# hrnr/map-merge

Measured on AMD Instinct MI355X. Metric: map-pairs/sec (normals+FPFH+SAC-IA+ICP, end to end incl. per-map features), higher is better.
Workload: dtype f32; 1 GPU; 16 maps x 500000 raw pts, FPFH + SAC_IA + ICP refine, 120 pairs; parallelism=one mm3d_estimate_maps_transforms call, 16 streams inside the library, points_after_filter_mean=406681, keypoints_mean=15692

## Files before the change

include/mm3d.h:

```cpp
#ifndef MM3D_H_
#define MM3D_H_

#include <stddef.h>
#include <stdint.h>

#ifdef __cplusplus
extern "C" {
#endif

typedef enum {
  MM3D_OK = 0,
  MM3D_EINVAL = -1,
  MM3D_EDEVICE = -2,
  MM3D_ENOMEM = -3,
  MM3D_EUNSUPPORTED = -4,
  MM3D_ECAPACITY = -5
} mm3d_status;

typedef enum { MM3D_DESC_PFH = 0, MM3D_DESC_PFHRGB, MM3D_DESC_FPFH, MM3D_DESC_RSD, MM3D_DESC_SHOT, MM3D_DESC_SC3D } mm3d_descriptor;
typedef enum { MM3D_KP_SIFT = 0, MM3D_KP_HARRIS } mm3d_keypoint;
typedef enum { MM3D_EST_MATCHING = 0, MM3D_EST_SAC_IA } mm3d_estimation_method;
typedef enum { MM3D_ICP_POINT_TO_POINT = 0, MM3D_ICP_POINT_TO_PLANE = 1 } mm3d_icp_method;

const char *mm3d_descriptor_name(int d);
// ... 71 lines not shown
int mm3d_debug_feature_lds_cap(int cap);
void mm3d_debug_feature_overflow(long long out[8], int reset);
void mm3d_debug_sacia_stats(long long out[4], int reset, int collect);
int mm3d_debug_desc_knn(mm3d_ctx *ctx, const float *a, size_t na, const float *b, size_t nb, int dim, int k, int *idx, float *d2);
typedef struct mm3d_nn_search_info {
  float max_d2;
  float rmax;
  float cell;
  float origin[3];
  int dims[3];
  int max_ring;
  int n_items;
} mm3d_nn_search_info;
int mm3d_debug_nn_search(mm3d_ctx *ctx, const mm3d_cloud *source, const mm3d_cloud *target, const float T[16], double range,
                         int convention, int split, int *idx, float *d2, mm3d_nn_search_info *info);
void mm3d_srand(mm3d_ctx *ctx, unsigned seed);
int mm3d_set_streams(mm3d_ctx *ctx, int n_streams);
int mm3d_get_streams(const mm3d_ctx *ctx);
int mm3d_last_run_stage_seconds(const mm3d_ctx *ctx, double *features_s, double *total_s);
int mm3d_last_run_device_seconds(const mm3d_ctx *ctx, double *exchange_s, double *pairs_s, double *gather_s);
size_t mm3d_last_run_map_sizes(const mm3d_ctx *ctx, size_t *points, size_t *keypoints, size_t capacity);
int mm3d_set_map_cache(mm3d_ctx *ctx, int max_maps);
int mm3d_get_map_cache(const mm3d_ctx *ctx);
void mm3d_map_cache_clear(mm3d_ctx *ctx);
int mm3d_map_cache_stats(const mm3d_ctx *ctx, long long out[6], int reset);
int mm3d_set_icp_method(mm3d_ctx *ctx, int method);
int mm3d_get_icp_method(const mm3d_ctx *ctx);
typedef enum { MM3D_ALIGN_SAC_IA = 0, MM3D_ALIGN_PREREJECTIVE = 1 } mm3d_align_method;
typedef struct mm3d_alignment_options {
  int method;
// ... 422 lines not shown
```

map-merge_amd/__init__.py:

```python
from __future__ import annotations

import ctypes as C
import enum
import os
import subprocess

import numpy as np

_HERE = os.path.dirname(os.path.abspath(__file__))
LIB_PATH = os.environ.get("MM3D_LIB") or os.path.join(_HERE, "libmm3d.so")

POINT = np.dtype([("x", "<f4"), ("y", "<f4"), ("z", "<f4"), ("rgba", "<u4")])
NORMAL = np.dtype([("nx", "<f4"), ("ny", "<f4"), ("nz", "<f4"), ("curvature", "<f4")])
CORR = np.dtype([("index_query", "<i4"), ("index_match", "<i4"), ("distance", "<f4")])
PAIR = np.dtype([("source_idx", "<u8"), ("target_idx", "<u8"), ("transform", "<f4", (16,)),
                 ("confidence", "<f8"), ("icp_iterations", "<i4"), ("n_correspondences", "<i4"),
                 ("n_inliers", "<i4"), ("icp_correspondences", "<i4")])


class Mm3dError(RuntimeError):
    def __init__(self, status, msg):
        super().__init__(f"mm3d status {status}: {msg}")
        self.status = status

# ... 1236 lines not shown
        self._ck(lib().mm3d_debug_wave_primitives(self._h, int(op), v.ctypes.data_as(C.c_void_p), len(v),
                                                  new.ctypes.data_as(C.c_void_p), old.ctypes.data_as(C.c_void_p)))
        return new, old

    def debugNnSearch(self, source_points, target_points, transform, range, convention, split):
        n = len(source_points)
        idx = np.zeros(max(n, 1), dtype=np.int32)
        d2 = np.zeros(max(n, 1), dtype=np.float32)
        t = _T(transform)
        info = NnSearchInfo()
        self._ck(lib().mm3d_debug_nn_search(self._h, source_points._h, target_points._h, t.ctypes.data_as(C.c_void_p),
                                            C.c_double(range), int(convention), int(split), idx.ctypes.data_as(C.c_void_p),
                                            d2.ctypes.data_as(C.c_void_p), C.byref(info)))
        return idx[:n], d2[:n], info.as_dict()

    def debugColorGradients(self, points, normals, options=None, **kw):
        o = options if options is not None else IcpColorOptions(**kw)
        n = len(points)
        out = np.zeros((max(n, 1), 4), dtype=np.float32)
        self._ck(lib().mm3d_debug_color_gradients(self._h, points._h, normals._h, C.byref(o), out.ctypes.data_as(C.c_void_p)))
        return out[:n]

    def debugIcpRejection(self, source_points, target_points, transform, max_correspondence_distance, options=None, split=1, **kw):
        o = options if options is not None else IcpRejectionOptions(**kw)
        n = len(source_points)
        idx = np.zeros(max(n, 1), dtype=np.int32)
        d2 = np.zeros(max(n, 1), dtype=np.float32)
        kept = np.zeros(max(n, 1), dtype=np.uint8)
        t = _T(transform)
        st = IcpRejectionStats()
# ... 247 lines not shown
```

map-merge_amd/csrc/device_util.hpp:

```cpp
#pragma once

#include <hip/hip_runtime.h>

#include <type_traits>

#include "libm_exact.hpp"
#include "types.hpp"

namespace mm3d {

constexpr int kWave = 64;
constexpr int kXcds = 8;

__device__ __forceinline__ unsigned xcd_remap(unsigned bid, unsigned nblocks)
{
  unsigned q = nblocks / kXcds, r = nblocks % kXcds;
  unsigned xcd = bid % kXcds, k = bid / kXcds;
  unsigned base = xcd < r ? xcd * (q + 1) : r * (q + 1) + (xcd - r) * q;
  return base + k;
}

__device__ __forceinline__ unsigned f2ord(float f)
{
  unsigned u = __float_as_uint(f);
// ... 14 lines not shown
__device__ __forceinline__ float dist2(float ax, float ay, float az, float bx, float by, float bz)
{
  float dx = ax - bx, dy = ay - by, dz = az - bz;
  return __fadd_rn(__fadd_rn(__fmul_rn(dx, dx), __fmul_rn(dy, dy)), __fmul_rn(dz, dz));
}

__device__ __forceinline__ float3 xform(const float *T, float x, float y, float z)
{
  float3 r;
  r.x = __fadd_rn(__fadd_rn(__fadd_rn(__fmul_rn(T[0], x), __fmul_rn(T[4], y)), __fmul_rn(T[8], z)), T[12]);
  r.y = __fadd_rn(__fadd_rn(__fadd_rn(__fmul_rn(T[1], x), __fmul_rn(T[5], y)), __fmul_rn(T[9], z)), T[13]);
  r.z = __fadd_rn(__fadd_rn(__fadd_rn(__fmul_rn(T[2], x), __fmul_rn(T[6], y)), __fmul_rn(T[10], z)), T[14]);
  return r;
}

__device__ __forceinline__ int cell_floor(float v, float mn, float inv)
{
  float f = floorf((v - mn) * inv);
  f = fminf(fmaxf(f, -1048576.0f), 1048576.0f);
  return (int)f;
}

__device__ __forceinline__ int clampi(int v, int lo, int hi) { return v < lo ? lo : (v > hi ? hi : v); }

template <class F>
__device__ __forceinline__ void for_each_candidate(const GridView &g, float qx, float qy, float qz, float r, F &&f)
{
  const float ri = r * 1.0001f + 1e-4f;
  int x0 = clampi(cell_floor(qx - ri, g.minx, g.inv), 0, g.dx - 1);
  int x1 = clampi(cell_floor(qx + ri, g.minx, g.inv), 0, g.dx - 1);
  int y0 = cell_floor(qy - ri, g.miny, g.inv), y1 = cell_floor(qy + ri, g.miny, g.inv);
  int z0 = cell_floor(qz - ri, g.minz, g.inv), z1 = cell_floor(qz + ri, g.minz, g.inv);
  if (cell_floor(qx + ri, g.minx, g.inv) < 0 || cell_floor(qx - ri, g.minx, g.inv) > g.dx - 1) return;
  y0 = y0 < 0 ? 0 : y0; z0 = z0 < 0 ? 0 : z0;
  y1 = y1 > g.dy - 1 ? g.dy - 1 : y1; z1 = z1 > g.dz - 1 ? g.dz - 1 : z1;
  for (int z = z0; z <= z1; ++z)
    for (int y = y0; y <= y1; ++y) {
      const int row = (z * g.dy + y) * g.dx;
// ... 368 lines not shown
```

map-merge_amd/csrc/filters.hip:

```cpp
#include <algorithm>
#include <climits>

#include "lattice.hpp"
#include "scan_fused.hpp"

namespace mm3d {

__global__ void k_voxel_keys(const float4 *__restrict__ pts, int n, float inv, int minbx, int minby, int minbz,
                             int mul1, int mul2, uint32_t *__restrict__ keys, uint32_t *__restrict__ vals)
{
  int i = blockIdx.x * blockDim.x + threadIdx.x;
  if (i >= n) return;
  float4 p = pts[i];
  vals[i] = (uint32_t)i;
  if (!(isfinite(p.x) && isfinite(p.y) && isfinite(p.z))) { keys[i] = 0xFFFFFFFFu; return; }
  int ijk0 = (int)(lattice_index(p.x, inv) - (float)minbx);
  int ijk1 = (int)(lattice_index(p.y, inv) - (float)minby);
  int ijk2 = (int)(lattice_index(p.z, inv) - (float)minbz);
  keys[i] = (uint32_t)(ijk0 + ijk1 * mul1 + ijk2 * mul2);
}

struct VoxelHeadLoad {
  const uint32_t *keys; int n;
  __device__ __forceinline__ int operator()(size_t j) const
  {
    if (j >= (size_t)n) return 0;
    const uint32_t k = keys[j];
    return (k != 0xFFFFFFFFu && (j == 0 || keys[j - 1] != k)) ? 1 : 0;
  }
};
struct VoxelStartStore {
  int n; int *starts; int *n_voxels;
  __device__ __forceinline__ void operator()(size_t j, int prefix, int v) const
  {
// ... 102 lines not shown
{
  auto *in = const_cast<mm3d_cloud *>(in_);
  cloud_bbox(c, in);
  const int n = (int)in->n;
  if (n == 0 || in->n_finite == 0) return cloud_from_device(c, DevBuf<float4>(c, 0), 0);
  const float leaf = (float)resolution;
  const VoxelSetup vs = voxel_setup(in, leaf);
  const float inv = vs.inv;
  if (vs.overflow) {
    DevBuf<float4> copy(c, in->n);
    MM3D_HIP(hipMemcpyAsync(copy.get(), in->pts.get(), in->n * 16, hipMemcpyDeviceToDevice, c->stream));
    return cloud_from_device(c, std::move(copy), in->n);
  }
  const int *min_b = vs.min_b, *div_b = vs.div_b;
  const int mul1 = div_b[0], mul2 = div_b[0] * div_b[1];
  DevBuf<uint32_t> keys(c, n), vals(c, n), keys2(c, n), vals2(c, n);
  MM3D_LAUNCH(c, "voxel_keys", n * 24.0, k_voxel_keys, dim3(div_up(n, 256)), dim3(256), 0, in->pts.get(), n, inv,
              min_b[0], min_b[1], min_b[2], mul1, mul2, keys.get(), vals.get());
  DevBuf<int> too_long(c, 1);
  counting_sort_pairs_u32(c, keys.get(), n, (uint64_t)div_b[0] * (uint64_t)div_b[1] * (uint64_t)div_b[2], keys2.get(), vals2.get(),
                          too_long.get(), in->n_finite == in->n);
  const size_t bound = in->n_finite;
  DevBuf<int> starts(c, (size_t)n + 1);
  static const unsigned cblocks_cap = [] { const char *e = getenv("MM3D_VOXEL_BLOCKS"); return e ? (unsigned)std::max(1, atoi(e)) : 240u; }();
  const unsigned cblocks = std::min<unsigned>(div_up(bound, 256), cblocks_cap);
  DevBuf<unsigned> ctl(c, 16 + 8 * (size_t)cblocks);
  DevBuf<float4> out(c, bound);
  const size_t ctl_bytes = (16 + 8 * (size_t)cblocks) * sizeof(unsigned);
  unsigned *h = (unsigned *)c->pin(64 + ctl_bytes);
  for (int attempt = 0; attempt < 2; ++attempt) {
    scan_fused(c, "voxel_starts", n * 12.0, (size_t)n + 1, VoxelHeadLoad{keys2.get(), n}, VoxelStartStore{n, starts.get(), (int *)ctl.get()});
    MM3D_LAUNCH(c, "voxel_centroid", in->n_finite * 32.0, k_voxel_centroid, dim3(cblocks), dim3(256), 0, in->pts.get(),
                (const uint32_t *)vals2.get(), (const int *)starts.get(), (int *)ctl.get(), attempt == 0 ? (const int *)too_long.get() : (const int *)nullptr, (int)in->n_finite, 2.0f * leaf,
                out.get(), ctl.get() + 16);
    MM3D_HIP(hipMemcpyAsync(h + 16, ctl.get(), ctl_bytes, hipMemcpyDeviceToHost, c->stream));
    MM3D_HIP(hipMemcpyAsync(h + 15, too_long.get(), sizeof(int), hipMemcpyDeviceToHost, c->stream));
    c->sync();
    if (attempt == 1 || !h[15]) break;
    sort_pairs_u32(c, keys.get(), keys2.get(), vals.get(), vals2.get(), n, 32);
  }
  const size_t nvox = h[16];
  refit_points(c, out, nvox, bound);
  mm3d_cloud *res = cloud_from_device(c, std::move(out), nvox);
  unsigned box[8];
  box_of_slots(h + 32, cblocks, box);
  cloud_set_bbox(res, box);
  if (h[17] == 0) res->voxel_leaf = leaf;
  c->settle();
  return res;
}

__global__ void __launch_bounds__(256)
k_radius_count(GridView g, float radius, float thr, int need, int *__restrict__ keep )
{
// ... 76 lines not shown
```

map-merge_amd/csrc/grid.hip:

```cpp
#include <hip/hip_runtime.h>

#include <cstring>

#include <rocprim/rocprim.hpp>

#include "device_util.hpp"
#include "scan_fused.hpp"

namespace mm3d {


__global__ void __launch_bounds__(256)
k_scan_int(const int *__restrict__ in, int *__restrict__ out, size_t n, unsigned long long *status, unsigned *ticket,
           unsigned ticket_base, unsigned epoch)
{
  __shared__ unsigned s_tile;
  __shared__ int s_wave[4];
  __shared__ int s_prefix;
  if (threadIdx.x == 0) s_tile = atomicAdd(ticket, 1u) - ticket_base;
  __syncthreads();
  const size_t tile = s_tile;
  const size_t base = tile * kScanTile + (size_t)threadIdx.x * kScanItems;
  int v[kScanItems];
  int sum = 0;
// ... 504 lines not shown
  MM3D_HIP(hipMemcpyAsync(h, g.nb_start.get() + nc, sizeof(int), hipMemcpyDeviceToHost, c->stream));
  c->sync();
  const size_t total = (size_t)h[0];
  g.nb_pts = DevBuf<float4>(c, total ? total : 1);
  if (total) {
    MM3D_LAUNCH(c, "grid_nblists", total * 32.0, k_nb_fill, dim3(div_up(nc, 4)), dim3(256), 0, (const int *)g.cell_start.get(),
                (const float4 *)g.sorted.get(), g.dims[0], g.dims[1], g.dims[2], R, (const int *)g.nb_start.get(), g.nb_pts.get());
    MM3D_LAUNCH(c, "grid_nblists", total * 32.0, k_nb_sort, dim3(div_up(nc, 4)), dim3(256), 0, g.mn[0], g.mn[1], g.mn[2], g.cell,
                g.dims[0], g.dims[1], g.dims[2], (const int *)g.nb_start.get(), g.nb_pts.get());
  }
  g.nb_R = R;
  c->settle();
}

__global__ void k_hilbert_keys(const float4 *__restrict__ pts, int n, float minx, float miny, float minz, float inv,
                               uint32_t *__restrict__ keys, uint32_t *__restrict__ vals, int *__restrict__ counts, uint32_t *__restrict__ ranks)
{
  const int i = blockIdx.x * blockDim.x + threadIdx.x;
  if (i >= n) return;
  const float4 p = pts[i];
  vals[i] = (uint32_t)i;
  if (!(isfinite(p.x) && isfinite(p.y) && isfinite(p.z))) { keys[i] = 0xFFFFFFFFu; return; }
  unsigned x = (unsigned)clampi(cell_floor(p.x, minx, inv), 0, 1023);
  unsigned y = (unsigned)clampi(cell_floor(p.y, miny, inv), 0, 1023);
  const unsigned z = (unsigned)clampi(cell_floor(p.z, minz, inv), 0, 1023);
  unsigned d = 0;
  for (unsigned sft = 512; sft > 0; sft >>= 1) {
    const unsigned rx = (x & sft) ? 1u : 0u, ry = (y & sft) ? 1u : 0u;
    d += sft * sft * ((3u * rx) ^ ry);
    if (ry == 0) {
      if (rx == 1) { x = 1023u - x; y = 1023u - y; }
      const unsigned t = x; x = y; y = t;
    }
  }
  const uint32_t key = (d << 10) | z;
  keys[i] = key;
  if (counts) ranks[i] = (uint32_t)atomicAdd(&counts[key >> 10], 1);
}

// ... 2 lines not shown
  const int j = blockIdx.x * blockDim.x + threadIdx.x;
  if (j >= n) return;
  const uint32_t i = order[j];
  float4 p = pts[i];
  p.w = __int_as_float((int)i);
  out[j] = p;
}

struct ItemHeadLoad {
  const uint32_t *keys; int n; const int *inert;
  __device__ __forceinline__ bool head(size_t j) const { return j < (size_t)n && (j == 0 || (keys[j] >> 16) != (keys[j - 1] >> 16) || (j & 63) == 0); }
  __device__ __forceinline__ int operator()(size_t j) const { return (inert && *inert) ? 0 : (head(j) ? 1 : 0); }
};
struct ItemFillStore {
  const uint32_t *keys; int n; int2 *items; int *n_items; const int *inert;
  __device__ __forceinline__ void operator()(size_t j, int prefix, int v) const
  {
    if (j == (size_t)n) { *n_items = prefix; return; }
    if (!v) return;
    const ItemHeadLoad h{keys, n, nullptr};
    int cnt = 1;
    while (cnt < 64 && j + cnt < (size_t)n && !h.head(j + cnt)) ++cnt;
    items[prefix] = make_int2((int)j, cnt);
  }
  __device__ __forceinline__ void done() const {}
};

constexpr int kCountSortBinMax = 1024;
__global__ void k_cs_count(const uint32_t *__restrict__ keys, int n, uint32_t divisor, int *__restrict__ counts, uint32_t *__restrict__ ranks)
{
  const int i = blockIdx.x * blockDim.x + threadIdx.x;
  if (i >= n) return;
  const uint32_t key = keys[i];
  if (key == 0xFFFFFFFFu) return;
  ranks[i] = (uint32_t)atomicAdd(&counts[key / divisor], 1);
}
__global__ void k_cs_scatter(const uint32_t *__restrict__ keys, const uint32_t *__restrict__ ranks, const int *__restrict__ bin_start, int n,
                             uint32_t divisor, int *__restrict__ slots, int *__restrict__ too_long)
{
  const int i = blockIdx.x * blockDim.x + threadIdx.x;
  if (i >= n) return;
  const uint32_t key = keys[i];
  if (key == 0xFFFFFFFFu) return;
  const uint32_t bin = key / divisor;
  const int b = bin_start[bin];
  slots[b + (int)ranks[i]] = i;
  if (bin_start[bin + 1] - b > kCountSortBinMax) *too_long = 1;
}
__global__ void k_cs_place(const uint32_t *__restrict__ keys, const int *__restrict__ bin_start, const int *__restrict__ slots, int n,
                           uint32_t divisor, const int *__restrict__ too_long, uint32_t *__restrict__ keys_out, uint32_t *__restrict__ idx_out)
{
  const int i = blockIdx.x * blockDim.x + threadIdx.x;
  if (i >= n || *too_long) return;
  const uint32_t key = keys[i];
  if (key == 0xFFFFFFFFu) return;
  const uint32_t bin = key / divisor;
  const int b = bin_start[bin], e = bin_start[bin + 1];
  int r = 0;
  for (int j = b; j < e; ++j) {
    const int o = slots[j];
    const uint32_t ko = keys[o];
    r += (ko < key || (ko == key && o < i)) ? 1 : 0;
  }
  keys_out[b + r] = key;
  idx_out[b + r] = (uint32_t)i;
}

void counting_sort_pairs_u32(Context *c, const uint32_t *keys, int n, uint64_t key_range, uint32_t *keys_out, uint32_t *idx_out,
                             int *too_long, bool no_invalid_keys)
{
  uint32_t divisor = (uint32_t)((key_range + ((uint64_t)1 << 22) - 1) >> 22);
  if (divisor == 0) divisor = 1;
  const int nbins = (int)(key_range / divisor) + 1;
  DevBuf<int> counts(c, (size_t)nbins + 1), bin_start(c, (size_t)nbins + 1), slots(c, (size_t)n);
  DevBuf<uint32_t> ranks(c, (size_t)n);
  MM3D_HIP(hipMemsetAsync(counts.get(), 0, ((size_t)nbins + 1) * sizeof(int), c->stream));
  MM3D_HIP(hipMemsetAsync(too_long, 0, sizeof(int), c->stream));
  if (!no_invalid_keys) MM3D_HIP(hipMemsetAsync(keys_out, 0xFF, (size_t)n * sizeof(uint32_t), c->stream));
  MM3D_LAUNCH(c, "count_sort", n * 12.0, k_cs_count, dim3(div_up(n, 256)), dim3(256), 0, keys, n, divisor, counts.get(), ranks.get());
  exclusive_scan_int(c, counts.get(), bin_start.get(), (size_t)nbins + 1);
  MM3D_LAUNCH(c, "count_sort", n * 16.0, k_cs_scatter, dim3(div_up(n, 256)), dim3(256), 0, keys, (const uint32_t *)ranks.get(),
              (const int *)bin_start.get(), n, divisor, slots.get(), too_long);
  MM3D_LAUNCH(c, "count_sort", n * 24.0, k_cs_place, dim3(div_up(n, 256)), dim3(256), 0, keys, (const int *)bin_start.get(),
              (const int *)slots.get(), n, divisor, (const int *)too_long, keys_out, idx_out);
}

constexpr int kHilColumns = 1 << 20;
constexpr int kHilColumnMax = 1024;
__global__ void k_hil_scatter(const uint32_t *__restrict__ keys, const uint32_t *__restrict__ ranks, const int *__restrict__ col_start, int n,
                              int *__restrict__ slots, int *__restrict__ too_long)
{
  const int i = blockIdx.x * blockDim.x + threadIdx.x;
  if (i >= n) return;
  const uint32_t key = keys[i];
  if (key == 0xFFFFFFFFu) return;
  const int b = col_start[key >> 10];
  slots[b + (int)ranks[i]] = i;
  if (col_start[(key >> 10) + 1] - b > kHilColumnMax) *too_long = 1;
}
__global__ void k_hil_place(const float4 *__restrict__ pts, const uint32_t *__restrict__ keys, const int *__restrict__ col_start,
                            const int *__restrict__ slots, int n, const int *__restrict__ too_long, float4 *__restrict__ out,
                            uint32_t *__restrict__ out_keys)
{
  const int i = blockIdx.x * blockDim.x + threadIdx.x;
  if (i >= n || *too_long) return;
  const uint32_t key = keys[i];
  if (key == 0xFFFFFFFFu) return;
  const int b = col_start[key >> 10], e = col_start[(key >> 10) + 1];
  int r = 0;
  for (int j = b; j < e; ++j) {
    const int o = slots[j];
    const uint32_t ko = keys[o];
    r += (ko < key || (ko == key && o < i)) ? 1 : 0;
  }
  float4 p = pts[i];
  p.w = __int_as_float(i);
  out[b + r] = p;
  out_keys[b + r] = key;
}

void cloud_hilbert(Context *c, const mm3d_cloud *cl_, float min_cell)
{
  auto *cl = const_cast<mm3d_cloud *>(cl_);
  std::lock_guard<std::recursive_mutex> lk(cl->cache_mu);
  cloud_bbox(c, cl);
  const int n = (int)cl->n_finite;
  if (cl->hil_pts.get() || n == 0) return;
  const int total = (int)cl->n;
  float ext = 0.f;
  for (int a = 0; a < 3; ++a) ext = std::fmax(ext, cl->bmax[a] - cl->bmin[a]);
  const float cell = std::fmax(std::fmax(0.25f, min_cell), ext / 1023.0f);
  DevBuf<uint32_t> keys(c, total), vals(c, total), keys2(c, total);
  cl->hil_pts = DevBuf<float4>(c, n);
  DevBuf<int> counts(c, kHilColumns + 2), col_start(c, kHilColumns + 1), slots(c, n);
  DevBuf<uint32_t> ranks(c, total);
  MM3D_HIP(hipMemsetAsync(counts.get(), 0, (kHilColumns + 2) * sizeof(int), c->stream));
  const DevPtr<int> too_long{counts.get() + kHilColumns + 1};
  MM3D_LAUNCH(c, "hilbert_keys", total * 36.0, k_hilbert_keys, dim3(div_up(total, 256)), dim3(256), 0, cl->pts.get(), total,
              cl->bmin[0], cl->bmin[1], cl->bmin[2], 1.0f / cell, keys.get(), vals.get(), counts.get(), ranks.get());
  exclusive_scan_int(c, counts.get(), col_start.get(), kHilColumns + 1);
  MM3D_LAUNCH(c, "hilbert_sort", total * 16.0, k_hil_scatter, dim3(div_up(total, 256)), dim3(256), 0, (const uint32_t *)keys.get(),
              (const uint32_t *)ranks.get(), (const int *)col_start.get(), total, slots.get(), too_long.get());
  MM3D_LAUNCH(c, "hilbert_sort", total * 44.0, k_hil_place, dim3(div_up(total, 256)), dim3(256), 0, cl->pts.get(),
              (const uint32_t *)keys.get(), (const int *)col_start.get(), (const int *)slots.get(), total, (const int *)too_long.get(),
              cl->hil_pts.get(), keys2.get());
  const size_t max_items = (size_t)n / 64 + 16384 + 2;
  cl->wave_items = DevBuf<int2>(c, max_items);
  DevBuf<int> n_items_dev(c, 1);
  int *h = (int *)c->pin(64);
  for (int attempt = 0; attempt < 2; ++attempt) {
    const int *inert = attempt == 0 ? (const int *)too_long.get() : nullptr;
    scan_fused(c, "hilbert_items", n * 20.0, (size_t)n + 1, ItemHeadLoad{keys2.get(), n, inert},
               ItemFillStore{keys2.get(), n, cl->wave_items.get(), n_items_dev.get(), inert});
    MM3D_HIP(hipMemcpyAsync(h, n_items_dev.get(), sizeof(int), hipMemcpyDeviceToHost, c->stream));
    MM3D_HIP(hipMemcpyAsync(h + 1, too_long.get(), sizeof(int), hipMemcpyDeviceToHost, c->stream));
    c->sync();
    if (attempt == 1 || !h[1]) break;
    DevBuf<uint32_t> vals2(c, total);
    sort_pairs_u32(c, keys.get(), keys2.get(), vals.get(), vals2.get(), total, 32);
// ... 73 lines not shown
}

int snb_cu_count(int device)
{
  static std::mutex mu;
  static std::map<int, int> cache;
  std::lock_guard<std::mutex> lk(mu);
  auto it = cache.find(device);
  if (it != cache.end()) return it->second;
  int n = 0;
  if (hipDeviceGetAttribute(&n, hipDeviceAttributeMultiprocessorCount, device) != hipSuccess || n <= 0) n = 256;
  cache[device] = n;
  return n;
}

}
```

map-merge_amd/csrc/scan_fused.hpp:

```cpp
#pragma once

#include "device_util.hpp"

namespace mm3d {

struct BoxAcc {
  float mn[3] = {INFINITY, INFINITY, INFINITY}, mx[3] = {-INFINITY, -INFINITY, -INFINITY};
  int cnt = 0;
  __device__ __forceinline__ void add(const float4 &p)
  {
    mn[0] = fminf(mn[0], p.x); mn[1] = fminf(mn[1], p.y); mn[2] = fminf(mn[2], p.z);
    mx[0] = fmaxf(mx[0], p.x); mx[1] = fmaxf(mx[1], p.y); mx[2] = fmaxf(mx[2], p.z);
    ++cnt;
  }
  template <bool kSlot>
  __device__ __forceinline__ void flush_impl(unsigned *box)
  {
    __shared__ float s_mn[4][3], s_mx[4][3];
    __shared__ int s_cnt[4];
#pragma unroll
    for (int a = 0; a < 3; ++a) { mn[a] = wave_min_f(mn[a]); mx[a] = wave_max_f(mx[a]); }
    const int total = wave_sum(cnt);
    const int lane = threadIdx.x & 63, wave = (threadIdx.x >> 6) & 3;
    if (lane == 0) {
// ... 23 lines not shown
  __device__ __forceinline__ void flush(unsigned *box) { flush_impl<false>(box); }
  __device__ __forceinline__ void flush_slot(unsigned *slots) { flush_impl<true>(slots + 8 * (size_t)blockIdx.x); }
};
inline void box_of_slots(const unsigned *slots, unsigned blocks, unsigned *box)
{
  for (int a = 0; a < 3; ++a) { box[a] = 0xFFFFFFFFu; box[3 + a] = 0u; }
  box[6] = 0u;
  for (unsigned b = 0; b < blocks; ++b) {
    const unsigned *s = slots + 8 * (size_t)b;
    for (int a = 0; a < 3; ++a) { box[a] = s[a] < box[a] ? s[a] : box[a]; box[3 + a] = s[3 + a] > box[3 + a] ? s[3 + a] : box[3 + a]; }
    box[6] += s[6];
  }
}
constexpr unsigned kBoxInit[8] = {0xFFFFFFFFu, 0xFFFFFFFFu, 0xFFFFFFFFu, 0u, 0u, 0u, 0u, 0u};

template <class Load, class Store>
__global__ void __launch_bounds__(256)
k_scan_fused(size_t n, unsigned long long *status, unsigned *ticket, unsigned ticket_base, unsigned epoch, Load load, Store store)
{
  __shared__ unsigned s_tile;
  __shared__ int s_wave[4];
  __shared__ int s_prefix;
  if (threadIdx.x == 0) s_tile = atomicAdd(ticket, 1u) - ticket_base;
  __syncthreads();
  const size_t tile = s_tile;
  const size_t base = tile * kScanTile + (size_t)threadIdx.x * kScanItems;
  int v[kScanItems];
  int sum = 0;
#pragma unroll
  for (int k = 0; k < kScanItems; ++k) v[k] = base + k < n ? load(base + k) : 0;
#pragma unroll
  for (int k = 0; k < kScanItems; ++k) sum += v[k];
  const int lane = threadIdx.x & 63, wave = threadIdx.x >> 6;
  const int incl = wave_scan_incl(sum);
  if (lane == kWave - 1) s_wave[wave] = incl;
  __syncthreads();
  int wave_off = 0;
  for (int w = 0; w < wave; ++w) wave_off += s_wave[w];
  const int total = s_wave[0] + s_wave[1] + s_wave[2] + s_wave[3];
  if (wave == 0) {
    const unsigned long long tag = (unsigned long long)epoch << 34;
    if (lane == 0 && tile > 0)
      __hip_atomic_store(&status[tile], tag | (1ull << 32) | (unsigned)total, __ATOMIC_RELAXED, __HIP_MEMORY_SCOPE_AGENT);
    int prefix = 0;
    for (long long hi = (long long)tile - 1; hi >= 0; hi -= kWave) {
      const long long t = hi - lane;
      unsigned long long w = 2ull << 32;
      if (t >= 0) {
// ... 1 lines not shown
        while ((w >> 34) != epoch || ((w >> 32) & 3u) == 0u);
      }
      const unsigned long long is_prefix = ballot(((w >> 32) & 3u) == 2u);
      const int first = __ffsll((long long)is_prefix) - 1;
      const int take = (first < 0 || lane <= first) ? (int)(unsigned)(w & 0xffffffffull) : 0;
      prefix += wave_sum(take);
      if (first >= 0) break;
    }
    if (lane == 0) {
      __hip_atomic_store(&status[tile], tag | (2ull << 32) | (unsigned)(prefix + total), __ATOMIC_RELAXED, __HIP_MEMORY_SCOPE_AGENT);
      s_prefix = prefix;
    }
  }
  __syncthreads();
  int run = s_prefix + wave_off + incl - sum;
#pragma unroll
  for (int k = 0; k < kScanItems; ++k) {
    if (base + k < n) store(base + k, run, v[k]);
    run += v[k];
  }
  store.done();
}

template <class Load, class Store>
void scan_fused(Context *c, const char *name, double bytes, size_t n, Load load, Store store)
{
  if (n == 0) return;
  const ScanLaunchState st = scan_prepare(c, n);
  MM3D_LAUNCH(c, name, bytes, (k_scan_fused<Load, Store>), dim3(st.tiles), dim3(256), 0, n, st.status, st.ticket, st.ticket_base, st.epoch, load, store);
}

}
```

map-merge_amd/csrc/types.hpp:

```cpp
#pragma once

#include "common.hpp"

namespace mm3d {
struct DeviceSet;
struct IcpMethodBase;
struct AlignMethodBase;
struct KeypointSourceBase;
struct CoarseMethodBase;
struct ConfidenceMethodBase;
struct EstimatorMethodBase;
struct IcpSamplerBase;
struct OutlierFilterBase;
struct ClusterFilterBase;
struct SmootherBase;
struct PlaneFilterBase;

struct StageSelection {
  const IcpMethodBase *icp = nullptr;
  const AlignMethodBase *align = nullptr;
  const KeypointSourceBase *keypoints = nullptr;
  const IcpMethodBase *refine = nullptr;
  const CoarseMethodBase *coarse = nullptr;
  const ConfidenceMethodBase *confidence = nullptr;
// ... 220 lines not shown
void cloud_hilbert(Context *c, const mm3d_cloud *cl, float min_cell = 0.25f);
mm3d_cloud *cloud_from_device(Context *c, DevBuf<float4> &&pts, size_t n);
mm3d_cloud *cloud_from_memory(Context *c, const void *src, size_t n, size_t stride, size_t rgba_off);
void cloud_download(Context *c, const mm3d_cloud *cl, void *dst, size_t stride, size_t rgba_off);
const std::vector<float4> &cloud_host(Context *c, const mm3d_cloud *cl, bool wait = true);
size_t compact_points(Context *c, const float4 *in, const int *flags, size_t n, DevBuf<float4> &out, unsigned *box_host = nullptr);
void cloud_set_bbox(mm3d_cloud *cl, const unsigned box[7]);
void refit_points(Context *c, DevBuf<float4> &out, size_t m, size_t bound);
mm3d_cloud *cloud_of_kept(Context *c, const mm3d_cloud *in, const int *flags, bool inherits_leaf, size_t *kept = nullptr);
void exclusive_scan_int(Context *c, const int *in, int *out, size_t n);
constexpr int kScanItems = 16, kScanTile = 256 * kScanItems;
struct ScanLaunchState { unsigned long long *status; unsigned *ticket; unsigned ticket_base, epoch, tiles; };
ScanLaunchState scan_prepare(Context *c, size_t n);
void counting_sort_pairs_u32(Context *c, const uint32_t *keys, int n, uint64_t key_range, uint32_t *keys_out, uint32_t *idx_out,
                             int *too_long, bool no_invalid_keys = false);
void sort_pairs_u32(Context *c, const uint32_t *kin, uint32_t *kout, const uint32_t *vin, uint32_t *vout,
                    size_t n, int end_bit);

mm3d_cloud *downsample(Context *c, const mm3d_cloud *in, double resolution);
bool downsample_is_identity(Context *c, const mm3d_cloud *in, double resolution);
mm3d_cloud *remove_outliers(Context *c, const mm3d_cloud *in, double radius, int min_neighbours);
mm3d_cloud *transform_concat(Context *c, const mm3d_cloud *const *clouds, size_t n, const float *T);

mm3d_normals *compute_normals(Context *c, const mm3d_cloud *in, double radius);

mm3d_cloud *detect_keypoints_sift(Context *c, const mm3d_cloud *points, double min_scale, int nr_octaves, int nr_scales, double min_contrast,
                                  double normals_radius = 0.0, mm3d_normals **normals_out = nullptr, float grid_cell_hint = 0.0f);
void normals_of_items(Context *c, const mm3d_cloud *in, const Grid &g, double radius, const int *ov_items, const int *ov_count_dev, int n_overflow,
                      float4 *out);

// ... 205 lines not shown
```

Baseline: 1464 map-pairs/s.

## Fuse voxel key counting, store key pairs in sort slots, precompute item spans

```diff
diff --git a/include/mm3d.h b/include/mm3d.h
--- a/include/mm3d.h
+++ b/include/mm3d.h
@@ -109,6 +109,9 @@
 } mm3d_nn_search_info;
 int mm3d_debug_nn_search(mm3d_ctx *ctx, const mm3d_cloud *source, const mm3d_cloud *target, const float T[16], double range,
                          int convention, int split, int *idx, float *d2, mm3d_nn_search_info *info);
+int mm3d_debug_hilbert_order(mm3d_ctx *ctx, const mm3d_cloud *cloud, float min_cell, int *order, int *items, size_t items_cap, int *n_items);
+int mm3d_debug_counting_sort(mm3d_ctx *ctx, const uint32_t *keys, size_t n, uint64_t key_range, int no_invalid_keys, uint32_t *keys_out,
+                             uint32_t *idx_out, int *too_long);
 void mm3d_srand(mm3d_ctx *ctx, unsigned seed);
 int mm3d_set_streams(mm3d_ctx *ctx, int n_streams);
 int mm3d_get_streams(const mm3d_ctx *ctx);
diff --git a/map-merge_amd/__init__.py b/map-merge_amd/__init__.py
--- a/map-merge_amd/__init__.py
+++ b/map-merge_amd/__init__.py
@@ -1274,6 +1274,26 @@
                                             d2.ctypes.data_as(C.c_void_p), C.byref(info)))
         return idx[:n], d2[:n], info.as_dict()
 
+    def debugHilbertOrder(self, points, min_cell=0.25):
+        n = len(points)
+        cap = n // 64 + 16386
+        order = np.full(max(n, 1), -1, dtype=np.int32)
+        items = np.zeros((cap, 2), dtype=np.int32)
+        m = C.c_int(0)
+        self._ck(lib().mm3d_debug_hilbert_order(self._h, points._h, C.c_float(min_cell), order.ctypes.data_as(C.c_void_p),
+                                                items.ctypes.data_as(C.c_void_p), C.c_size_t(cap), C.byref(m)))
+        order = order[:n]
+        return order[order >= 0], items[:m.value]
+
+    def debugCountingSort(self, keys, key_range, no_invalid_keys=False):
+        k = np.ascontiguousarray(keys, dtype=np.uint32)
+        ko, io = np.zeros(len(k), dtype=np.uint32), np.zeros(len(k), dtype=np.uint32)
+        tl = C.c_int(0)
+        self._ck(lib().mm3d_debug_counting_sort(self._h, k.ctypes.data_as(C.c_void_p), C.c_size_t(len(k)), C.c_uint64(int(key_range)),
+                                                int(bool(no_invalid_keys)), ko.ctypes.data_as(C.c_void_p), io.ctypes.data_as(C.c_void_p),
+                                                C.byref(tl)))
+        return ko, io, bool(tl.value)
+
     def debugColorGradients(self, points, normals, options=None, **kw):
         o = options if options is not None else IcpColorOptions(**kw)
         n = len(points)
diff --git a/map-merge_amd/csrc/device_util.hpp b/map-merge_amd/csrc/device_util.hpp
--- a/map-merge_amd/csrc/device_util.hpp
+++ b/map-merge_amd/csrc/device_util.hpp
@@ -52,14 +52,14 @@
   return r;
 }
 
-__device__ __forceinline__ int cell_floor(float v, float mn, float inv)
+__host__ __device__ __forceinline__ int cell_floor(float v, float mn, float inv)
 {
   float f = floorf((v - mn) * inv);
   f = fminf(fmaxf(f, -1048576.0f), 1048576.0f);
   return (int)f;
 }
 
-__device__ __forceinline__ int clampi(int v, int lo, int hi) { return v < lo ? lo : (v > hi ? hi : v); }
+__host__ __device__ __forceinline__ int clampi(int v, int lo, int hi) { return v < lo ? lo : (v > hi ? hi : v); }
 
 template <class F>
 __device__ __forceinline__ void for_each_candidate(const GridView &g, float qx, float qy, float qz, float r, F &&f)
diff --git a/map-merge_amd/csrc/filters.hip b/map-merge_amd/csrc/filters.hip
--- a/map-merge_amd/csrc/filters.hip
+++ b/map-merge_amd/csrc/filters.hip
@@ -18,6 +18,21 @@
   int ijk1 = (int)(lattice_index(p.y, inv) - (float)minby);
   int ijk2 = (int)(lattice_index(p.z, inv) - (float)minbz);
   keys[i] = (uint32_t)(ijk0 + ijk1 * mul1 + ijk2 * mul2);
+}
+
+__global__ void k_voxel_keys_count(const float4 *__restrict__ pts, int n, float inv, int minbx, int minby, int minbz, int mul1, int mul2,
+                                   uint32_t divisor, uint32_t *__restrict__ keys, int *__restrict__ counts, uint32_t *__restrict__ ranks)
+{
+  int i = blockIdx.x * blockDim.x + threadIdx.x;
+  if (i >= n) return;
+  float4 p = pts[i];
+  if (!(isfinite(p.x) && isfinite(p.y) && isfinite(p.z))) { keys[i] = 0xFFFFFFFFu; return; }
+  int ijk0 = (int)(lattice_index(p.x, inv) - (float)minbx);
+  int ijk1 = (int)(lattice_index(p.y, inv) - (float)minby);
+  int ijk2 = (int)(lattice_index(p.z, inv) - (float)minbz);
+  const uint32_t key = (uint32_t)(ijk0 + ijk1 * mul1 + ijk2 * mul2);
+  keys[i] = key;
+  if (key != 0xFFFFFFFFu) ranks[i] = (uint32_t)atomicAdd(&counts[key / divisor], 1);
 }
 
 struct VoxelHeadLoad {
@@ -150,12 +165,21 @@
   }
   const int *min_b = vs.min_b, *div_b = vs.div_b;
   const int mul1 = div_b[0], mul2 = div_b[0] * div_b[1];
+  const uint64_t key_range = (uint64_t)div_b[0] * (uint64_t)div_b[1] * (uint64_t)div_b[2];
+#if MM3D_VOXEL_FUSED
+  DevBuf<uint32_t> keys(c, n), keys2(c, n), vals2(c, n);
+  const CountingSort cs = counting_sort_begin(c, n, key_range);
+  const DevPtr<int> too_long{cs.too_long()};
+  MM3D_LAUNCH(c, "voxel_keys", n * 28.0, k_voxel_keys_count, dim3(div_up(n, 256)), dim3(256), 0, in->pts.get(), n, inv,
+              min_b[0], min_b[1], min_b[2], mul1, mul2, cs.divisor, keys.get(), cs.counts.get(), cs.ranks.get());
+  counting_sort_finish(c, cs, keys.get(), n, keys2.get(), vals2.get(), in->n_finite == in->n);
+#else
   DevBuf<uint32_t> keys(c, n), vals(c, n), keys2(c, n), vals2(c, n);
   MM3D_LAUNCH(c, "voxel_keys", n * 24.0, k_voxel_keys, dim3(div_up(n, 256)), dim3(256), 0, in->pts.get(), n, inv,
               min_b[0], min_b[1], min_b[2], mul1, mul2, keys.get(), vals.get());
   DevBuf<int> too_long(c, 1);
-  counting_sort_pairs_u32(c, keys.get(), n, (uint64_t)div_b[0] * (uint64_t)div_b[1] * (uint64_t)div_b[2], keys2.get(), vals2.get(),
-                          too_long.get(), in->n_finite == in->n);
+  counting_sort_pairs_u32(c, keys.get(), n, key_range, keys2.get(), vals2.get(), too_long.get(), in->n_finite == in->n);
+#endif
   const size_t bound = in->n_finite;
   DevBuf<int> starts(c, (size_t)n + 1);
   static const unsigned cblocks_cap = [] { const char *e = getenv("MM3D_VOXEL_BLOCKS"); return e ? (unsigned)std::max(1, atoi(e)) : 240u; }();
@@ -173,7 +197,14 @@
     MM3D_HIP(hipMemcpyAsync(h + 15, too_long.get(), sizeof(int), hipMemcpyDeviceToHost, c->stream));
     c->sync();
     if (attempt == 1 || !h[15]) break;
+#if MM3D_VOXEL_FUSED
+    DevBuf<uint32_t> vals(c, n);
+    iota_u32(c, vals.get(), n);
+#endif
     sort_pairs_u32(c, keys.get(), keys2.get(), vals.get(), vals2.get(), n, 32);
+#if MM3D_VOXEL_FUSED
+    c->settle();
+#endif
   }
   const size_t nvox = h[16];
   refit_points(c, out, nvox, bound);
diff --git a/map-merge_amd/csrc/grid.hip b/map-merge_amd/csrc/grid.hip
--- a/map-merge_amd/csrc/grid.hip
+++ b/map-merge_amd/csrc/grid.hip
@@ -1,9 +1,12 @@
 #include <hip/hip_runtime.h>
 
+#include <cmath>
 #include <cstring>
+#include <vector>
 
 #include <rocprim/rocprim.hpp>
 
+#include "capi_guard.hpp"
 #include "device_util.hpp"
 #include "scan_fused.hpp"
 
@@ -542,15 +545,16 @@
 }
 
 __global__ void k_hilbert_keys(const float4 *__restrict__ pts, int n, float minx, float miny, float minz, float inv,
-                               uint32_t *__restrict__ keys, uint32_t *__restrict__ vals, int *__restrict__ counts, uint32_t *__restrict__ ranks)
+                               uint32_t *__restrict__ keys, uint32_t *__restrict__ vals, int *__restrict__ counts, uint32_t *__restrict__ ranks,
+                               int col_max )
 {
   const int i = blockIdx.x * blockDim.x + threadIdx.x;
   if (i >= n) return;
   const float4 p = pts[i];
   vals[i] = (uint32_t)i;
   if (!(isfinite(p.x) && isfinite(p.y) && isfinite(p.z))) { keys[i] = 0xFFFFFFFFu; return; }
-  unsigned x = (unsigned)clampi(cell_floor(p.x, minx, inv), 0, 1023);
-  unsigned y = (unsigned)clampi(cell_floor(p.y, miny, inv), 0, 1023);
+  unsigned x = (unsigned)clampi(cell_floor(p.x, minx, inv), 0, col_max);
+  unsigned y = (unsigned)clampi(cell_floor(p.y, miny, inv), 0, col_max);
   const unsigned z = (unsigned)clampi(cell_floor(p.z, minz, inv), 0, 1023);
   unsigned d = 0;
   for (unsigned sft = 512; sft > 0; sft >>= 1) {
@@ -583,6 +587,14 @@
 };
 struct ItemFillStore {
   const uint32_t *keys; int n; int2 *items; int *n_items; const int *inert;
+#if MM3D_ITEM_NEXT
+  static constexpr bool kNextFlag = true;
+  __device__ __forceinline__ void operator()(size_t j, int prefix, int v, int next) const
+  {
+    if (j == (size_t)n) { *n_items = prefix; return; }
+    if (v) items[prefix] = make_int2((int)j, min(next, n - (int)j));
+  }
+#else
   __device__ __forceinline__ void operator()(size_t j, int prefix, int v) const
   {
     if (j == (size_t)n) { *n_items = prefix; return; }
@@ -592,6 +604,7 @@
     while (cnt < 64 && j + cnt < (size_t)n && !h.head(j + cnt)) ++cnt;
     items[prefix] = make_int2((int)j, cnt);
   }
+#endif
   __device__ __forceinline__ void done() const {}
 };
 
@@ -604,8 +617,43 @@
   if (key == 0xFFFFFFFFu) return;
   ranks[i] = (uint32_t)atomicAdd(&counts[key / divisor], 1);
 }
+#if MM3D_PLACE_PAIRS
+typedef uint2 SortSlot;
+__device__ __forceinline__ SortSlot sort_slot(uint32_t key, int i) { return make_uint2(key, (uint32_t)i); }
+__device__ __forceinline__ int sort_rank(const SortSlot *__restrict__ slots, const uint32_t *, int b, int e, uint32_t key, int i)
+{
+  const uint32_t ui = (uint32_t)i;
+  int r = 0, j = b;
+  for (; j + 4 <= e; j += 4) {
+    const uint2 m0 = slots[j], m1 = slots[j + 1], m2 = slots[j + 2], m3 = slots[j + 3];
+    r += (m0.x < key || (m0.x == key && m0.y < ui)) ? 1 : 0;
+    r += (m1.x < key || (m1.x == key && m1.y < ui)) ? 1 : 0;
+    r += (m2.x < key || (m2.x == key && m2.y < ui)) ? 1 : 0;
+    r += (m3.x < key || (m3.x == key && m3.y < ui)) ? 1 : 0;
+  }
+  for (; j < e; ++j) {
+    const uint2 m = slots[j];
+    r += (m.x < key || (m.x == key && m.y < ui)) ? 1 : 0;
+  }
+  return r;
+}
+#else
+typedef int SortSlot;
+__device__ __forceinline__ SortSlot sort_slot(uint32_t, int i) { return i; }
+__device__ __forceinline__ int sort_rank(const SortSlot *__restrict__ slots, const uint32_t *__restrict__ keys, int b, int e, uint32_t key, int i)
+{
+  int r = 0;
+  for (int j = b; j < e; ++j) {
+    const int o = slots[j];
+    const uint32_t ko = keys[o];
+    r += (ko < key || (ko == key && o < i)) ? 1 : 0;
+  }
+  return r;
+}
+#endif
+
 __global__ void k_cs_scatter(const uint32_t *__restrict__ keys, const uint32_t *__restrict__ ranks, const int *__restrict__ bin_start, int n,
-                             uint32_t divisor, int *__restrict__ slots, int *__restrict__ too_long)
+                             uint32_t divisor, SortSlot *__restrict__ slots, int *__restrict__ too_long)
 {
   const int i = blockIdx.x * blockDim.x + threadIdx.x;
   if (i >= n) return;
@@ -613,10 +661,10 @@
   if (key == 0xFFFFFFFFu) return;
   const uint32_t bin = key / divisor;
   const int b = bin_start[bin];
-  slots[b + (int)ranks[i]] = i;
+  slots[b + (int)ranks[i]] = sort_slot(key, i);
   if (bin_start[bin + 1] - b > kCountSortBinMax) *too_long = 1;
 }
-__global__ void k_cs_place(const uint32_t *__restrict__ keys, const int *__restrict__ bin_start, const int *__restrict__ slots, int n,
+__global__ void k_cs_place(const uint32_t *__restrict__ keys, const int *__restrict__ bin_start, const SortSlot *__restrict__ slots, int n,
                            uint32_t divisor, const int *__restrict__ too_long, uint32_t *__restrict__ keys_out, uint32_t *__restrict__ idx_out)
 {
   const int i = blockIdx.x * blockDim.x + threadIdx.x;
@@ -625,50 +673,80 @@
   if (key == 0xFFFFFFFFu) return;
   const uint32_t bin = key / divisor;
   const int b = bin_start[bin], e = bin_start[bin + 1];
-  int r = 0;
-  for (int j = b; j < e; ++j) {
-    const int o = slots[j];
-    const uint32_t ko = keys[o];
-    r += (ko < key || (ko == key && o < i)) ? 1 : 0;
-  }
+  const int r = sort_rank(slots, keys, b, e, key, i);
   keys_out[b + r] = key;
   idx_out[b + r] = (uint32_t)i;
 }
 
+static uint32_t counting_sort_divisor(uint64_t key_range)
+{
+  const uint32_t divisor = (uint32_t)((key_range + ((uint64_t)1 << 22) - 1) >> 22);
+  return divisor == 0 ? 1 : divisor;
+}
+
+static void counting_sort_place(Context *c, const uint32_t *keys, const uint32_t *ranks, const int *counts, int nbins, uint32_t divisor, int n,
+                                uint32_t *keys_out, uint32_t *idx_out, int *too_long)
+{
+  DevBuf<int> bin_start(c, (size_t)nbins + 1);
+  DevBuf<SortSlot> slots(c, (size_t)n);
+  exclusive_scan_int(c, counts, bin_start.get(), (size_t)nbins + 1);
+  MM3D_LAUNCH(c, "count_sort", n * 16.0, k_cs_scatter, dim3(div_up(n, 256)), dim3(256), 0, keys, ranks,
+              (const int *)bin_start.get(), n, divisor, slots.get(), too_long);
+  MM3D_LAUNCH(c, "count_sort", n * 24.0, k_cs_place, dim3(div_up(n, 256)), dim3(256), 0, keys, (const int *)bin_start.get(),
+              (const SortSlot *)slots.get(), n, divisor, (const int *)too_long, keys_out, idx_out);
+}
+
 void counting_sort_pairs_u32(Context *c, const uint32_t *keys, int n, uint64_t key_range, uint32_t *keys_out, uint32_t *idx_out,
                              int *too_long, bool no_invalid_keys)
 {
-  uint32_t divisor = (uint32_t)((key_range + ((uint64_t)1 << 22) - 1) >> 22);
-  if (divisor == 0) divisor = 1;
+  const uint32_t divisor = counting_sort_divisor(key_range);
   const int nbins = (int)(key_range / divisor) + 1;
-  DevBuf<int> counts(c, (size_t)nbins + 1), bin_start(c, (size_t)nbins + 1), slots(c, (size_t)n);
+  DevBuf<int> counts(c, (size_t)nbins + 1);
   DevBuf<uint32_t> ranks(c, (size_t)n);
   MM3D_HIP(hipMemsetAsync(counts.get(), 0, ((size_t)nbins + 1) * sizeof(int), c->stream));
   MM3D_HIP(hipMemsetAsync(too_long, 0, sizeof(int), c->stream));
   if (!no_invalid_keys) MM3D_HIP(hipMemsetAsync(keys_out, 0xFF, (size_t)n * sizeof(uint32_t), c->stream));
   MM3D_LAUNCH(c, "count_sort", n * 12.0, k_cs_count, dim3(div_up(n, 256)), dim3(256), 0, keys, n, divisor, counts.get(), ranks.get());
-  exclusive_scan_int(c, counts.get(), bin_start.get(), (size_t)nbins + 1);
-  MM3D_LAUNCH(c, "count_sort", n * 16.0, k_cs_scatter, dim3(div_up(n, 256)), dim3(256), 0, keys, (const uint32_t *)ranks.get(),
-              (const int *)bin_start.get(), n, divisor, slots.get(), too_long);
-  MM3D_LAUNCH(c, "count_sort", n * 24.0, k_cs_place, dim3(div_up(n, 256)), dim3(256), 0, keys, (const int *)bin_start.get(),
-              (const int *)slots.get(), n, divisor, (const int *)too_long, keys_out, idx_out);
+  counting_sort_place(c, keys, ranks.get(), counts.get(), nbins, divisor, n, keys_out, idx_out, too_long);
+}
+
+CountingSort counting_sort_begin(Context *c, int n, uint64_t key_range)
+{
+  CountingSort cs;
+  cs.divisor = counting_sort_divisor(key_range);
+  cs.nbins = (int)(key_range / cs.divisor) + 1;
+  cs.counts = DevBuf<int>(c, (size_t)cs.nbins + 2);
+  cs.ranks = DevBuf<uint32_t>(c, (size_t)n);
+  MM3D_HIP(hipMemsetAsync(cs.counts.get(), 0, ((size_t)cs.nbins + 2) * sizeof(int), c->stream));
+  return cs;
+}
+
+void counting_sort_finish(Context *c, const CountingSort &cs, const uint32_t *keys, int n, uint32_t *keys_out, uint32_t *idx_out, bool no_invalid_keys)
+{
+  if (!no_invalid_keys) MM3D_HIP(hipMemsetAsync(keys_out, 0xFF, (size_t)n * sizeof(uint32_t), c->stream));
+  counting_sort_place(c, keys, cs.ranks.get(), cs.counts.get(), cs.nbins, cs.divisor, n, keys_out, idx_out, cs.too_long());
+}
+
+void iota_u32(Context *c, uint32_t *v, int n)
+{
+  if (n > 0) MM3D_LAUNCH(c, "iota", n * 4.0, k_iota_u32, dim3(div_up(n, 256)), dim3(256), 0, v, n);
 }
 
 constexpr int kHilColumns = 1 << 20;
 constexpr int kHilColumnMax = 1024;
 __global__ void k_hil_scatter(const uint32_t *__restrict__ keys, const uint32_t *__restrict__ ranks, const int *__restrict__ col_start, int n,
-                              int *__restrict__ slots, int *__restrict__ too_long)
+                              SortSlot *__restrict__ slots, int *__restrict__ too_long)
 {
   const int i = blockIdx.x * blockDim.x + threadIdx.x;
   if (i >= n) return;
   const uint32_t key = keys[i];
   if (key == 0xFFFFFFFFu) return;
   const int b = col_start[key >> 10];
-  slots[b + (int)ranks[i]] = i;
+  slots[b + (int)ranks[i]] = sort_slot(key, i);
   if (col_start[(key >> 10) + 1] - b > kHilColumnMax) *too_long = 1;
 }
 __global__ void k_hil_place(const float4 *__restrict__ pts, const uint32_t *__restrict__ keys, const int *__restrict__ col_start,
-                            const int *__restrict__ slots, int n, const int *__restrict__ too_long, float4 *__restrict__ out,
+                            const SortSlot *__restrict__ slots, int n, const int *__restrict__ too_long, float4 *__restrict__ out,
                             uint32_t *__restrict__ out_keys)
 {
   const int i = blockIdx.x * blockDim.x + threadIdx.x;
@@ -676,12 +754,7 @@
   const uint32_t key = keys[i];
   if (key == 0xFFFFFFFFu) return;
   const int b = col_start[key >> 10], e = col_start[(key >> 10) + 1];
-  int r = 0;
-  for (int j = b; j < e; ++j) {
-    const int o = slots[j];
-    const uint32_t ko = keys[o];
-    r += (ko < key || (ko == key && o < i)) ? 1 : 0;
-  }
+  const int r = sort_rank(slots, keys, b, e, key, i);
   float4 p = pts[i];
   p.w = __int_as_float(i);
   out[b + r] = p;
@@ -701,17 +774,26 @@
   const float cell = std::fmax(std::fmax(0.25f, min_cell), ext / 1023.0f);
   DevBuf<uint32_t> keys(c, total), vals(c, total), keys2(c, total);
   cl->hil_pts = DevBuf<float4>(c, n);
-  DevBuf<int> counts(c, kHilColumns + 2), col_start(c, kHilColumns + 1), slots(c, n);
+  const float inv = 1.0f / cell;
+  int col_bits = 10;
+#if MM3D_HIL_BOX
+  const int cmax = std::max(clampi(cell_floor(cl->bmax[0], cl->bmin[0], inv), 0, 1023), clampi(cell_floor(cl->bmax[1], cl->bmin[1], inv), 0, 1023));
+  for (col_bits = 0; (1 << col_bits) <= cmax; ++col_bits) {}
+#endif
+  const size_t ncol = (size_t)1 << (2 * col_bits);
+  static_assert(kHilColumns == 1 << 20, "ten bits per column coordinate");
+  DevBuf<int> counts(c, ncol + 2), col_start(c, ncol + 1);
+  DevBuf<SortSlot> slots(c, n);
   DevBuf<uint32_t> ranks(c, total);
-  MM3D_HIP(hipMemsetAsync(counts.get(), 0, (kHilColumns + 2) * sizeof(int), c->stream));
-  const DevPtr<int> too_long{counts.get() + kHilColumns + 1};
+  MM3D_HIP(hipMemsetAsync(counts.get(), 0, (ncol + 2) * sizeof(int), c->stream));
+  const DevPtr<int> too_long{counts.get() + ncol + 1};
   MM3D_LAUNCH(c, "hilbert_keys", total * 36.0, k_hilbert_keys, dim3(div_up(total, 256)), dim3(256), 0, cl->pts.get(), total,
-              cl->bmin[0], cl->bmin[1], cl->bmin[2], 1.0f / cell, keys.get(), vals.get(), counts.get(), ranks.get());
-  exclusive_scan_int(c, counts.get(), col_start.get(), kHilColumns + 1);
+              cl->bmin[0], cl->bmin[1], cl->bmin[2], inv, keys.get(), vals.get(), counts.get(), ranks.get(), (1 << col_bits) - 1);
+  exclusive_scan_int(c, counts.get(), col_start.get(), ncol + 1);
   MM3D_LAUNCH(c, "hilbert_sort", total * 16.0, k_hil_scatter, dim3(div_up(total, 256)), dim3(256), 0, (const uint32_t *)keys.get(),
               (const uint32_t *)ranks.get(), (const int *)col_start.get(), total, slots.get(), too_long.get());
   MM3D_LAUNCH(c, "hilbert_sort", total * 44.0, k_hil_place, dim3(div_up(total, 256)), dim3(256), 0, cl->pts.get(),
-              (const uint32_t *)keys.get(), (const int *)col_start.get(), (const int *)slots.get(), total, (const int *)too_long.get(),
+              (const uint32_t *)keys.get(), (const int *)col_start.get(), (const SortSlot *)slots.get(), total, (const int *)too_long.get(),
               cl->hil_pts.get(), keys2.get());
   const size_t max_items = (size_t)n / 64 + 16384 + 2;
   cl->wave_items = DevBuf<int2>(c, max_items);
@@ -815,4 +897,62 @@
   return n;
 }
 
-}
+static void debug_hilbert_order(Context *c, const mm3d_cloud *cl, float min_cell, int *order, int *items, size_t cap, int *n_items)
+{
+  MM3D_REQUIRE(!cl->hil_pts.get(), "mm3d_debug_hilbert_order: the cloud already carries an order");
+  cloud_hilbert(c, cl, min_cell);
+  for (size_t i = 0; i < cl->n; ++i) order[i] = -1;
+  *n_items = 0;
+  if (!cl->hil_pts.get()) return;
+  const size_t nf = cl->n_finite, ni = (size_t)cl->n_wave_items;
+  MM3D_REQUIRE(ni <= cap, "mm3d_debug_hilbert_order: more items than the caller's array holds");
+  std::vector<float4> h(nf);
+  MM3D_HIP(hipMemcpyAsync(h.data(), cl->hil_pts.get(), nf * sizeof(float4), hipMemcpyDeviceToHost, c->stream));
+  if (ni) MM3D_HIP(hipMemcpyAsync(items, cl->wave_items.get(), ni * sizeof(int2), hipMemcpyDeviceToHost, c->stream));
+  c->sync();
+  for (size_t j = 0; j < nf; ++j) std::memcpy(&order[j], &h[j].w, sizeof(int));
+  *n_items = (int)ni;
+}
+
+static void debug_counting_sort(Context *c, const uint32_t *keys, int n, uint64_t key_range, bool no_invalid_keys, uint32_t *keys_out,
+                                uint32_t *idx_out, int *too_long)
+{
+  DevBuf<uint32_t> d_keys(c, n), d_out(c, 2 * (size_t)n);
+  MM3D_HIP(hipMemcpyAsync(d_keys.get(), keys, (size_t)n * sizeof(uint32_t), hipMemcpyHostToDevice, c->stream));
+  MM3D_HIP(hipMemsetAsync(d_out.get(), 0xFF, 2 * (size_t)n * sizeof(uint32_t), c->stream));
+#if MM3D_VOXEL_FUSED
+  const CountingSort cs = counting_sort_begin(c, n, key_range);
+  const DevPtr<int> d_long{cs.too_long()};
+  MM3D_LAUNCH(c, "count_sort", n * 12.0, k_cs_count, dim3(div_up(n, 256)), dim3(256), 0, (const uint32_t *)d_keys.get(), n, cs.divisor,
+              cs.counts.get(), cs.ranks.get());
+  counting_sort_finish(c, cs, d_keys.get(), n, d_out.get(), d_out.get() + n, no_invalid_keys);
+#else
+  DevBuf<int> d_long(c, 1);
+  counting_sort_pairs_u32(c, d_keys.get(), n, key_range, d_out.get(), d_out.get() + n, d_long.get(), no_invalid_keys);
+#endif
+  MM3D_HIP(hipMemcpyAsync(keys_out, d_out.get(), (size_t)n * sizeof(uint32_t), hipMemcpyDeviceToHost, c->stream));
+  MM3D_HIP(hipMemcpyAsync(idx_out, d_out.get() + n, (size_t)n * sizeof(uint32_t), hipMemcpyDeviceToHost, c->stream));
+  MM3D_HIP(hipMemcpyAsync(too_long, d_long.get(), sizeof(int), hipMemcpyDeviceToHost, c->stream));
+  c->sync();
+}
+
+}
+
+extern "C" int mm3d_debug_hilbert_order(mm3d_ctx *ctx, const mm3d_cloud *cloud, float min_cell, int *order, int *items, size_t items_cap,
+                                        int *n_items)
+{
+  if (!cloud || !n_items || !(min_cell >= 0.0f) || !std::isfinite(min_cell)) return MM3D_EINVAL;
+  if ((cloud->n && !order) || (items_cap && !items)) return MM3D_EINVAL;
+  return mm3d::guarded(ctx, [&] { mm3d::debug_hilbert_order(ctx, cloud, min_cell, order, items, items_cap, n_items); });
+}
+
+extern "C" int mm3d_debug_counting_sort(mm3d_ctx *ctx, const uint32_t *keys, size_t n, uint64_t key_range, int no_invalid_keys,
+                                        uint32_t *keys_out, uint32_t *idx_out, int *too_long)
+{
+  if (!keys || !keys_out || !idx_out || !too_long || n == 0 || n > (size_t)1 << 30) return MM3D_EINVAL;
+  if (key_range == 0 || key_range > 0xFFFFFFFFull) return MM3D_EINVAL;
+  for (size_t i = 0; i < n; ++i) {
+    if (keys[i] == 0xFFFFFFFFu ? no_invalid_keys != 0 : keys[i] >= key_range) return MM3D_EINVAL;
+  }
+  return mm3d::guarded(ctx, [&] { mm3d::debug_counting_sort(ctx, keys, (int)n, key_range, no_invalid_keys != 0, keys_out, idx_out, too_long); });
+}
diff --git a/map-merge_amd/csrc/scan_fused.hpp b/map-merge_amd/csrc/scan_fused.hpp
--- a/map-merge_amd/csrc/scan_fused.hpp
+++ b/map-merge_amd/csrc/scan_fused.hpp
@@ -61,6 +61,11 @@
 }
 constexpr unsigned kBoxInit[8] = {0xFFFFFFFFu, 0xFFFFFFFFu, 0xFFFFFFFFu, 0u, 0u, 0u, 0u, 0u};
 
+template <class S, class = void> struct scan_store_wants_next : std::false_type {};
+template <class S> struct scan_store_wants_next<S, std::void_t<decltype(S::kNextFlag)>> : std::bool_constant<S::kNextFlag> {};
+constexpr int kScanNextSpan = 64;
+static_assert(kScanNextSpan == 4 * kScanItems, "the look-ahead is four runs: four mask words behind a thread's own");
+
 template <class Load, class Store>
 __global__ void __launch_bounds__(256)
 k_scan_fused(size_t n, unsigned long long *status, unsigned *ticket, unsigned ticket_base, unsigned epoch, Load load, Store store)
@@ -79,6 +84,19 @@
 #pragma unroll
   for (int k = 0; k < kScanItems; ++k) sum += v[k];
   const int lane = threadIdx.x & 63, wave = threadIdx.x >> 6;
+  constexpr bool kNext = scan_store_wants_next<Store>::value;
+  __shared__ unsigned s_mask[kNext ? 256 + 4 : 1];
+  unsigned mask = 0;
+  if constexpr (kNext) {
+#pragma unroll
+    for (int k = 0; k < kScanItems; ++k) mask |= v[k] ? 1u << k : 0u;
+    s_mask[threadIdx.x] = mask;
+    if (wave == 0) {
+      const size_t j = (tile + 1) * kScanTile + (size_t)lane;
+      const unsigned long long behind = ballot(j < n && load(j) != 0);
+      if (lane < 4) s_mask[256 + lane] = (unsigned)(behind >> (16 * lane)) & 0xffffu;
+    }
+  }
   const int incl = wave_scan_incl(sum);
   if (lane == kWave - 1) s_wave[wave] = incl;
   __syncthreads();
@@ -110,10 +128,28 @@
   }
   __syncthreads();
   int run = s_prefix + wave_off + incl - sum;
+  if constexpr (kNext) {
+    int after = kScanNextSpan;
+    if (mask) {
+      const unsigned long long m = (unsigned long long)s_mask[threadIdx.x + 1] | (unsigned long long)s_mask[threadIdx.x + 2] << 16 |
+                                   (unsigned long long)s_mask[threadIdx.x + 3] << 32 | (unsigned long long)s_mask[threadIdx.x + 4] << 48;
+      if (m) after = __ffsll((long long)m) - 1;
+    }
 #pragma unroll
-  for (int k = 0; k < kScanItems; ++k) {
-    if (base + k < n) store(base + k, run, v[k]);
-    run += v[k];
+    for (int k = 0; k < kScanItems; ++k) {
+      if (base + k < n) {
+        const unsigned later = k + 1 < kScanItems ? mask >> (k + 1) : 0u;
+        const int next = !v[k] ? 0 : (later ? __ffs((int)later) : min(kScanItems - k + after, kScanNextSpan));
+        store(base + k, run, v[k], next);
+      }
+      run += v[k];
+    }
+  } else {
+#pragma unroll
+    for (int k = 0; k < kScanItems; ++k) {
+      if (base + k < n) store(base + k, run, v[k]);
+      run += v[k];
+    }
   }
   store.done();
 }
diff --git a/map-merge_amd/csrc/types.hpp b/map-merge_amd/csrc/types.hpp
--- a/map-merge_amd/csrc/types.hpp
+++ b/map-merge_amd/csrc/types.hpp
@@ -258,6 +258,28 @@
 ScanLaunchState scan_prepare(Context *c, size_t n);
 void counting_sort_pairs_u32(Context *c, const uint32_t *keys, int n, uint64_t key_range, uint32_t *keys_out, uint32_t *idx_out,
                              int *too_long, bool no_invalid_keys = false);
+#ifndef MM3D_ITEM_NEXT
+#define MM3D_ITEM_NEXT 1
+#endif
+#ifndef MM3D_PLACE_PAIRS
+#define MM3D_PLACE_PAIRS 1
+#endif
+#ifndef MM3D_VOXEL_FUSED
+#define MM3D_VOXEL_FUSED 1
+#endif
+#ifndef MM3D_HIL_BOX
+#define MM3D_HIL_BOX 1
+#endif
+struct CountingSort {
+  uint32_t divisor = 1;
+  int nbins = 0;
+  DevBuf<int> counts;
+  DevBuf<uint32_t> ranks;
+  int *too_long() const { return counts.get() + nbins + 1; }
+};
+CountingSort counting_sort_begin(Context *c, int n, uint64_t key_range);
+void counting_sort_finish(Context *c, const CountingSort &cs, const uint32_t *keys, int n, uint32_t *keys_out, uint32_t *idx_out, bool no_invalid_keys);
+void iota_u32(Context *c, uint32_t *v, int n);
 void sort_pairs_u32(Context *c, const uint32_t *kin, uint32_t *kout, const uint32_t *vin, uint32_t *vout,
                     size_t n, int end_bit);
 
```

New measurement: 1480 map-pairs/s, median of 6. 1.01x the previous value.
